# Nikhil-AI-Labs/image-super-resolution-2

Measured on AMD Instinct MI355X. Metric: output MPix/s at x4 SR (256->1024), higher is better.
Workload: dtype bf16 (bf16 MFMA operands, fp32 accumulate, fp32 activations in HBM); 1 GPU; FreqFusion x4 full 3-expert forward (HAT-L + DAT + NAFNet-SR + fusion stack), one 256x256 LR tile -> 1024x1024 per step per GPU (BASELINE configs[1]); seeded synthetic weights (172.3 M params), 1/f-noise tiles; tile=256, parallelism=tile-sharded x1, weights RCCL-broadcast once (0.0 ms), no per-tile collectives, launch=hipGraph replay, tiles_in_flight=2

## Files before the change

### image-super-resolution-2_amd/build.py

```python
from __future__ import annotations

import os
import subprocess
import sys
from concurrent.futures import ThreadPoolExecutor

HERE = os.path.dirname(os.path.abspath(__file__))
CSRC = os.path.join(HERE, "csrc")
LIB = os.path.join(HERE, "libff_hip.so")
SOURCES = ["ff_runtime.hip", "conv_gemm.hip", "conv_gemm_bf16.hip", "conv3x3_halo.hip", "sgfn_tail.hip", "ocab_attn.hip", "conv3x3_small.hip", "attention.hip", "attention_bf16.hip", "win_attn_fused.hip", "chan_qkv.hip", "token_mlp.hip", "token_linear.hip", "naf_fused.hip", "naf_tail.hip", "norm_pool.hip", "dwconv.hip", "elementwise.hip",
           "resample.hip", "freq.hip", "fusion_ops.hip", "metrics.hip", "train_ops.hip", "sr_losses.hip", "augment.hip", "ff_executor.hip"]
HIPCC = os.environ.get("HIPCC", "/opt/rocm/bin/hipcc")
FLAGS = ["--offload-arch=gfx950", "-O3", "-fPIC", "-std=c++17", "-Wall", "-Wno-unused-function", "-I" + os.path.join(HERE, "build")]


def _stale() -> bool:
    if not os.path.exists(LIB):
        return True
    t = os.path.getmtime(LIB)
    deps = [os.path.join(CSRC, f) for f in os.listdir(CSRC)] + [os.path.join(HERE, "..", "include", "ff_kernels.h")]
    return any(os.path.getmtime(d) > t for d in deps)


def gen_dispatch(path: str) -> None:
    from .lib import parse_header
    protos = {n: p for n, p in parse_header().items() if p[1] and p[1][-1] == "void*" and p[0] == "int"
              and n not in ("ff_forward", "ff_create", "ff_upload")}
    names = sorted(protos)
    out = ["// generated by build.py from include/ff_kernels.h -- do not edit", f"#define FF_DISPATCH_COUNT {len(names)}",
           "static const char* const FF_DISPATCH_NAMES[FF_DISPATCH_COUNT] = {" + ", ".join(f'"{n}"' for n in names) + "};"]
    def kinds(n):
        ks = []
        for i, ty in enumerate(protos[n][1]):
            if i == len(protos[n][1]) - 1:
                ks.append("S")
            elif ty.endswith("*"):
                ks.append("P")
            elif ty in ("float", "double"):
                ks.append("F")
            else:
                ks.append("I")
        return "".join(ks)
    out.append("static const char* const FF_DISPATCH_KINDS[FF_DISPATCH_COUNT] = {" + ", ".join(f'"{kinds(n)}"' for n in names) + "};")
# ... 47 lines not shown
```

### image-super-resolution-2_amd/csrc/norm_pool.hip

```cpp
#include "ff_common.h"

template <int NV>
__global__ __launch_bounds__(256) void layernorm_kernel(const float* __restrict__ in, int ldi, float* __restrict__ out,
                                                        int ldo, int rows, int C, const float* __restrict__ g,
                                                        const float* __restrict__ bta, float eps) {
  const int lane = threadIdx.x & 63;
  const int row = blockIdx.x * 4 + (threadIdx.x >> 6);
  if (row >= rows) return;
  const float* x = in + (long long)row * ldi;
  float v[NV];
  float s = 0.f;
#pragma unroll
  for (int i = 0; i < NV; ++i) {
    const int c = lane + 64 * i;
    v[i] = c < C ? x[c] : 0.f;
    s += v[i];
  }
  const float mean = ff_wave_sum(s) / (float)C;
  float q = 0.f;
#pragma unroll
  for (int i = 0; i < NV; ++i) {
    const int c = lane + 64 * i;
    const float d = c < C ? v[i] - mean : 0.f;
    q += d * d;
  }
  const float rstd = 1.0f / sqrtf(ff_wave_sum(q) / (float)C + eps);
  float* y = out + (long long)row * ldo;
#pragma unroll
  for (int i = 0; i < NV; ++i) {
    const int c = lane + 64 * i;
    if (c < C) y[c] = (v[i] - mean) * rstd * g[c] + bta[c];
  }
}

extern "C" int ff_layernorm(const float* in, int ldi, float* out, int ldo, long long rows, int C, const float* gamma,
                            const float* beta, float eps, void* stream) {
  FF_CHECK_ARG(in && out && gamma && beta, "ff_layernorm: null pointer");
  FF_CHECK_ARG(C > 0 && C <= 1024 && ldi >= C && ldo >= C && rows > 0, "ff_layernorm: bad dims C=%d", C);
  FF_CHECK_ARG(rows < (1LL << 31), "ff_layernorm: too many rows");
  hipStream_t st = (hipStream_t)stream;
  dim3 grid((unsigned)((rows + 3) / 4)), block(256);
  const int nv = (C + 63) / 64;
#define LN_CASE(N) hipLaunchKernelGGL(layernorm_kernel<N>, grid, block, 0, st, in, ldi, out, ldo, (int)rows, C, gamma, beta, eps)
  if (nv <= 1) LN_CASE(1);
  else if (nv <= 2) LN_CASE(2);
  else if (nv <= 3) LN_CASE(3);
  else if (nv <= 4) LN_CASE(4);
  else if (nv <= 6) LN_CASE(6);
  else if (nv <= 8) LN_CASE(8);
  else LN_CASE(16);
#undef LN_CASE
  FF_LAUNCH_CHECK("ff_layernorm");
  return FF_OK;
}

__global__ __launch_bounds__(256) void pool_partial_v4_kernel(const float* __restrict__ in, int ld, long long P, int C,
                                                              int pix_per_chunk, float* __restrict__ part) {
  extern __shared__ float4 red4[];
  const int cv = C >> 2, rpi = 256 / cv;
  const int col = threadIdx.x % cv, row = threadIdx.x / cv;
  const int chunk = blockIdx.x, b = blockIdx.y, nch = gridDim.x;
  const long long p0 = (long long)chunk * pix_per_chunk;
  long long p1 = p0 + pix_per_chunk;
  if (p1 > P) p1 = P;
  const float* base = in + (long long)b * P * ld + 4 * col;
  float4 a0 = {0.f, 0.f, 0.f, 0.f}, a1 = a0, a2 = a0, a3 = a0;
  if (row < rpi) {
    long long pp = p0 + row;
    for (; pp + 3LL * rpi < p1; pp += 4LL * rpi) {
      const float4 v0 = *reinterpret_cast<const float4*>(base + pp * ld);
      const float4 v1 = *reinterpret_cast<const float4*>(base + (pp + rpi) * ld);
      const float4 v2 = *reinterpret_cast<const float4*>(base + (pp + 2LL * rpi) * ld);
      const float4 v3 = *reinterpret_cast<const float4*>(base + (pp + 3LL * rpi) * ld);
      a0.x += v0.x; a0.y += v0.y; a0.z += v0.z; a0.w += v0.w;
      a1.x += v1.x; a1.y += v1.y; a1.z += v1.z; a1.w += v1.w;
      a2.x += v2.x; a2.y += v2.y; a2.z += v2.z; a2.w += v2.w;
      a3.x += v3.x; a3.y += v3.y; a3.z += v3.z; a3.w += v3.w;
    }
    for (; pp < p1; pp += rpi) {
      const float4 v0 = *reinterpret_cast<const float4*>(base + pp * ld);
      a0.x += v0.x; a0.y += v0.y; a0.z += v0.z; a0.w += v0.w;
    }
    a0.x += a1.x + a2.x + a3.x; a0.y += a1.y + a2.y + a3.y; a0.z += a1.z + a2.z + a3.z; a0.w += a1.w + a2.w + a3.w;
    red4[row * cv + col] = a0;
  }
  __syncthreads();
// ... 332 lines not shown
```

### image-super-resolution-2_amd/experts.py

```python
from __future__ import annotations

from typing import Dict, List, Optional

import torch

from . import ops
from .prep import (pack_conv, pack_dw, bn_scale_shift, fold_bn_after_conv, pack_token_linear, pack_naf_ffn, pack_naf_tail,
                   pack_win_attn, pack_win_rel, pack_token_projmlp, pack_chan_qkv, pack_token_linear_gated, pack_rel_overlap)

T = torch.Tensor
SD = Dict[str, T]
RGB_MEAN = (0.4488, 0.4371, 0.4040)


def _ceil_to(n: int, m: int) -> int:
    return (n + m - 1) // m * m


class _Weights:

    def __init__(self, sd: SD, dev, prefix: str):
        self.sd, self.dev, self.p = sd, dev, prefix

    def __call__(self, name: str) -> T:
# ... 368 lines not shown
                 dec=(2, 2, 2, 2)):
        w = _Weights(sd, dev, prefix)
        self.dev, self.enc_n, self.mid_n, self.dec_n = dev, enc, mid, dec

        def blk(q):
            def c1(n):
                wt = w(q + n + ".weight")
                return wt.reshape(wt.shape[0], wt.shape[1]).contiguous(), w(q + n + ".bias")
            return dict(n1=(w(q + "norm1.weight"), w(q + "norm1.bias")), n2=(w(q + "norm2.weight"), w(q + "norm2.bias")),
                        c1=c1("conv1"), c2=(pack_dw(w(q + "conv2.weight")), w(q + "conv2.bias")), c3=c1("conv3"),
                        sca=c1("sca.1"), c4=c1("conv4"), c5=c1("conv5"),
                        beta=w(q + "beta").reshape(-1).contiguous(), gamma=w(q + "gamma").reshape(-1).contiguous())

        self.intro = (w.conv("intro"), w("intro.bias"))
        self.ending = (w.conv("ending"), w("ending.bias"))
        self.encs = [[blk(f"encoders.{l}.{b}.") for b in range(n)] for l, n in enumerate(enc)]
        self.mids = [blk(f"middle_blks.{b}.") for b in range(mid)]
        self.decs = [[blk(f"decoders.{l}.{b}.") for b in range(n)] for l, n in enumerate(dec)]
        self.downs = [(w.conv(f"downs.{l}"), w(f"downs.{l}.bias")) for l in range(len(enc))]
        self.ups = [w(f"ups.{l}.0.weight").reshape(w(f"ups.{l}.0.weight").shape[0], -1).contiguous() for l in range(len(dec))]

    def _padded_input(self, B: int, Hp: int, Wp: int, dev) -> T:
        return ops.persistent_zeros(id(self), "naf_in", (B, Hp, Wp, 3), dev)

    def __del__(self):
        try:
            ops.drop_persistent(owner=id(self))
        except Exception:
            pass

    def block(self, x: T, k: dict) -> T:
        c = x.shape[-1]
        flash = ops.fused_modes() and c in (64, 128)
        if flash and c == 64:
            g, pooled = ops.naf_front(x, _tl(k, "c1"), k["n1"][0], k["n1"][1], *k["c2"])
        else:
            if flash:
                t = ops.token_linear(x, _tl(k, "c1"), gamma=k["n1"][0], beta=k["n1"][1], eps=1e-6)
            else:
                t = ops.linear(ops.layernorm(x, *k["n1"], eps=1e-6), *k["c1"])
            g, pooled = ops.dwconv3_gate_pool(t, *k["c2"])
        sca = ops.vec_mlp(pooled, *k["sca"], None)
        if flash and ops.gemm_mode() == "bf16":
            if "tail_pk" not in k:
                k["tail_pk"] = pack_naf_tail(*k["c3"], *k["c4"], *k["c5"])
            return ops.naf_tail(g, x, k["tail_pk"], sca.reshape(-1), k["beta"], k["n2"][0], k["n2"][1], k["gamma"])
        nf = ops.gemm_mode() != "f32"
        if nf:
            y = ops.linear(g, *k["c3"], res=x, mul=k["beta"], kmul=sca.reshape(-1))
        else:
            w3 = ops.mix2(k["c3"][0], ca=sca.reshape(-1))
            y = ops.linear(g, w3, k["c3"][1], res=x, mul=k["beta"], dynamic_w=True)
        if flash:
            if "ffn_pk" not in k:
                k["ffn_pk"] = pack_naf_ffn(k["c4"][0], k["c4"][1], k["c5"][0], k["c5"][1])
            return ops.naf_ffn(y, k["ffn_pk"], k["n2"][0], k["n2"][1], k["gamma"])
        if nf:
            if "c4i" not in k:
                w4, b4 = k["c4"]
                k["c4i"] = (torch.stack((w4[:c], w4[c:]), dim=1).reshape(2 * c, -1).contiguous(),
                            torch.stack((b4[:c], b4[c:]), dim=1).reshape(-1).contiguous())
            g = ops.linear(ops.layernorm(y, *k["n2"], eps=1e-6), *k["c4i"], gate_pairs=True)
        else:
            t = ops.linear(ops.layernorm(y, *k["n2"], eps=1e-6), *k["c4"])
            g = ops.fma3(None, t[..., :c], t[..., c:])
        return ops.linear(g, *k["c5"], res=y, mul=k["gamma"])

    def forward(self, lr: T, taps: Optional[dict] = None, feats: Optional[dict] = None) -> T:
        _, _, h, w = lr.shape
        H, W = 4 * h, 4 * w
        m = 2 ** len(self.enc_n)
        Hp, Wp = _ceil_to(H, m), _ceil_to(W, m)
        inp = self._padded_input(1, Hp, Wp, lr.device)
        ops.resize(lr, (H, W), mode="bicubic", scale_factor=4.0, layout="nchw", out=inp)
        x = ops.conv2d(inp, *self.intro, ksize=(3, 3), pad=(1, 1))
        skips = []
        for lvl, blks in enumerate(self.encs):
            for b, k in enumerate(blks):
                x = self.block(x, k)
                if taps is not None and lvl == 0:
                    taps[f"naf.enc0.b{b}"] = x
            skips.append(x)
            x = ops.conv2d(x, *self.downs[lvl], ksize=(2, 2), stride=(2, 2), pad=(0, 0))
        for k in self.mids:
            x = self.block(x, k)
        if taps is not None:
            taps["naf.mid"] = x
        for lvl, blks in enumerate(self.decs):
            x = ops.conv2d(x, self.ups[lvl], None, shuffle=2, res=skips[-1 - lvl])
            for k in blks:
                x = self.block(x, k)
        if feats is not None:
            feats["nafnet"] = x
        x = ops.conv2d(x, *self.ending, ksize=(3, 3), pad=(1, 1), res=inp)
        return ops.nhwc_to_nchw(x, H, W, clamp01=True)
# ... 1 lines not shown
```

### image-super-resolution-2_amd/ops.py

```python
from __future__ import annotations

from typing import Dict, Optional, Tuple

import torch

from . import lib as _lib

ACT = {None: 0, "none": 0, "gelu": 1, "relu": 2, "lrelu": 3, "sigmoid": 4}
T = torch.Tensor

_PROF = None
_META = [0.0, 0.0]


def _note(flops: float = 0.0, nbytes: float = 0.0):
    _META[0] += flops
    _META[1] += nbytes


def _numel(*ts) -> float:
    return float(sum(t.numel() * (t.element_size() / 4.0) for t in ts if t is not None))


def _instrument(fn):
# ... 37 lines not shown
import os as _os

GEMM_MODES = {"f32": 0, "bf16": 1, "bf16x2": 2, "bf16x3": 3}
_GEMM_MODE = _os.environ.get("FF_GEMM", "bf16x3")


def set_gemm_mode(mode: str):
    global _GEMM_MODE
    if mode not in GEMM_MODES:
        raise _lib.FFError(f"unknown GEMM mode {mode!r}; expected one of {sorted(GEMM_MODES)}")
    _GEMM_MODE = mode


def _nterms() -> int:
    if _GEMM_MODE not in ("bf16x3", "bf16"):
        raise _lib.FFError(f"the fused bf16 kernels exist for the 'bf16x3' and 'bf16' contraction modes, not {_GEMM_MODE!r}")
    return 3 if _GEMM_MODE == "bf16x3" else 1


def fused_modes() -> bool:
    return _GEMM_MODE in ("bf16x3", "bf16")


def gemm_mode() -> str:
    return _GEMM_MODE


_HALO = True


def set_halo(on: bool) -> None:
    global _HALO
    _HALO = bool(on)


def empty_rows_bf16(shape, device) -> T:
    C = int(shape[-1])
    return torch.empty(tuple(shape[:-1]) + ((C + 63) // 64 * 64,), device=device, dtype=torch.bfloat16)[..., :C]


def empty_rows(shape, device) -> T:
    C = int(shape[-1])
    if C >= 48 and C % 32 != 0:
        return torch.empty(tuple(shape[:-1]) + ((C + 31) // 32 * 32,), device=device, dtype=torch.float32)[..., :C]
    return torch.empty(tuple(shape), device=device, dtype=torch.float32)


def empty_like_rows(x: T) -> T:
    return empty_rows(tuple(x.shape), x.device)


_LANE = 0


def lane() -> int:
    return _LANE


def set_lane(k: int) -> None:
    global _LANE
    _LANE = int(k)


_CAPTURE_KEY = None
_PERSIST_GRAPH: Dict[tuple, Dict[tuple, T]] = {}
_PERSIST_EAGER: Dict[tuple, T] = {}
# ... 210 lines not shown

        nt_ = _nterms()

        def _mk_halo():
            bn = _prep.halo_bn(Cout)
            return (_prep.pack_conv3x3_halo(w, Cin, bn, nt_), bn)
        img = PREPARED.get(w, "halo" if nt_ == 3 else "halo1", _mk_halo)
        part = None
        if want_pool and B == 1 and shuffle == 0 and Cout <= img[1]:
            prow = int(_L().ff_conv3x3_halo_pool_rows(B, H, W, Cout, img[1], nt_))
            part = torch.empty((prow, img[1]), device=x.device, dtype=torch.float32)
        _lib.check(_L().ff_conv3x3_halo(xp, ldi, img[0].data_ptr(), img[1], _ptr(bias), _ptr(mul), rp, ldr, op, ldo, B, H, W,
                                        Cin, Cout, ACT[act], float(alpha), shuffle, _ptr(part), _nterms(),
                                        (1 if in_bf16 else 0) | (2 if out_bf16 else 0), _stream()))
        if part is not None:
            pp = PoolPartials(part, Cout, 1.0 / float(H * W))
            _note(2.0 * B * Ho * Wo * Cout * KH * KW * Cin, 4.0 * (_numel(x, w, out, res)))
            return out, (pp if want_pool == "partials" else pp.mean())
    else:
        aligned = (ldi % 4 == 0) and (xp % 16 == 0)
        hi, lo, Kp, Cp, _ = _split_weight(w, dynamic_w, Cin if aligned else 0)
        _lib.check(_L().ff_conv2d_bf16s(xp, hi.data_ptr(), lo.data_ptr() if lo is not None else None, Kp, Cp, _ptr(bias), _ptr(mul),
                                        rp, op, B, H, W, Cin, ldi, Ho, Wo, Cout, ldo, ldr, KH, KW, stride[0], stride[1],
                                        pad[0], pad[1], ACT[act], float(alpha), shuffle, GEMM_MODES[_GEMM_MODE], tile_hint,
                                        None, _stream()))
    _note(2.0 * B * Ho * Wo * Cout * KH * KW * Cin, 4.0 * (_numel(x, w, out, res)))
    if want_pool:
        return out, pool_mean(out)
    return out


def linear(x: T, w: T, bias: Optional[T] = None, *, act=None, res: Optional[T] = None, mul: Optional[T] = None,
           alpha: float = 1.0, out: Optional[T] = None, dynamic_w: bool = False, kmul: Optional[T] = None,
           gate_pairs: bool = False) -> T:
    xp, ldi, rows, K = rows_view(x, "linear.x")
    N = w.shape[0]
    if w.dim() != 2 or w.shape[1] != K or not w.is_contiguous():
        raise _lib.FFError(f"linear: weight must be [N, {K}], got {tuple(w.shape)}")
    if (kmul is not None or gate_pairs) and _GEMM_MODE == "f32":
        raise _lib.FFError("linear: kmul / gate_pairs exist in the split-bf16 kernels only")
    No = N // 2 if gate_pairs else N
    oshape = tuple(x.shape[:-1]) + (No,)
    if out is None:
        out = empty_rows(oshape, x.device)
    op, ldo, orows, oc = rows_view(out, "linear.out")
    if orows != rows or oc != No:
        raise _lib.FFError("linear: out shape mismatch")
    rp, ldr = None, 0
    if res is not None:
        rp, ldr, rrows, rc = rows_view(res, "linear.res")
        if rrows != rows or rc != N:
            raise _lib.FFError("linear: res shape mismatch")
    if _GEMM_MODE == "f32":
        _lib.check(_L().ff_conv2d(xp, w.data_ptr(), _ptr(bias), _ptr(mul), rp, op, 1, 1, rows, K, ldi, 1, rows, N, ldo, ldr,
                                  1, 1, 1, 1, 0, 0, ACT[act], float(alpha), 0, 0, _stream()))
    else:
        aligned = (ldi % 4 == 0) and (xp % 16 == 0)
        hi, lo, Kp, Cp, _ = _split_weight(w, dynamic_w, K if aligned else 0)
        if kmul is not None and (kmul.numel() != K or not kmul.is_contiguous()):
            raise _lib.FFError(f"linear: kmul must be a contiguous [{K}] vector")
        _lib.check(_L().ff_conv2d_bf16s(xp, hi.data_ptr(), lo.data_ptr() if lo is not None else None, Kp, Cp, _ptr(bias), _ptr(mul),
                                        rp, op, 1, 1, rows, K, ldi, 1, rows, N, ldo, ldr, 1, 1, 1, 1, 0, 0, ACT[act],
                                        float(alpha), 1 if gate_pairs else 0, GEMM_MODES[_GEMM_MODE], 0, _ptr(kmul), _stream()))
    _note(2.0 * rows * N * K, 4.0 * (rows * K + N * K + rows * No * (2 if res is not None else 1)))
    return out


def window_attn(qkv: T, out: T, biasT: T, *, q_off: int, k_off: int, v_off: int, o_off: int, H: int, W: int, Hp: int,
                Wp: int, win: Tuple[int, int], kwin: Tuple[int, int], shift: Tuple[int, int], use_mask: bool, heads: int,
                d: int, scale: float, rel_table: Optional[T] = None) -> T:
    qp, ldq, B, h_, w_, _ = _nhwc(qkv, "window_attn.qkv")
    op, ldo, *_ = _nhwc(out, "window_attn.out")
    if (h_, w_) != (H, W) or tuple(out.shape[:3]) != (B, H, W):
        raise _lib.FFError("window_attn: qkv/out spatial dims mismatch")
    nk = kwin[0] * kwin[1]
    if tuple(biasT.shape) != (heads, nk, 256) or not biasT.is_contiguous():
        raise _lib.FFError(f"window_attn: biasT must be [{heads},{nk},256]")
    if q_off + heads * d > qkv.shape[-1] or k_off + heads * d > qkv.shape[-1] or v_off + heads * d > qkv.shape[-1] \
            or o_off + heads * d > out.shape[-1]:
        raise _lib.FFError("window_attn: channel offsets out of range")
    if _GEMM_MODE == "f32":
        _lib.check(_L().ff_window_attn(qp, ldq, q_off, k_off, v_off, op, ldo, o_off, biasT.data_ptr(), B, H, W, Hp, Wp, win[0],
                                       win[1], kwin[0], kwin[1], shift[0], shift[1], int(use_mask), heads, d, float(scale),
                                       _stream()))
    else:
        relp = None
        if rel_table is not None and tuple(kwin) != tuple(win):
            n = (win[0] + kwin[0] - 1) * (win[1] + kwin[1] - 1)
            if tuple(rel_table.shape) != (heads, n) or not rel_table.is_contiguous() or kwin[1] % 8 or tuple(shift) != (0, 0):
                raise _lib.FFError(f"window_attn: overlapping-window rel_table must be [heads, {n}] (prep.pack_rel_overlap), kw % 8 == 0, no shift")
            relp = rel_table.data_ptr()
        elif rel_table is not None and tuple(kwin) == tuple(win) and win[1] & (win[1] - 1) == 0 and win[1] >= 8:
            if tuple(rel_table.shape) != (heads, (2 * win[0] - 1) * (2 * win[1] - 1)) or not rel_table.is_contiguous():
                raise _lib.FFError("window_attn: rel_table must be [heads, (2wh-1)*(2ww-1)]")
            relp = rel_table.data_ptr()
        from . import prep as _prep
        bq = PREPARED.get(biasT, "quad", lambda: _prep.quad_bias(biasT))
# ... 163 lines not shown
    return out, pooled


def naf_ffn(y: T, pk: dict, ln_g: T, ln_b: T, out_scale: T, eps: float = 1e-6) -> T:
    yp, ldy, rows, C = rows_view(y, "naf_ffn.y")
    if C != pk["C"]:
        raise _lib.FFError("naf_ffn: channel mismatch")
    out = torch.empty(tuple(y.shape), device=y.device, dtype=torch.float32)
    _lib.check(_L().ff_naf_ffn(yp, ldy, out.data_ptr(), C, rows, C, ln_g.data_ptr(), ln_b.data_ptr(), float(eps), pk["w"].data_ptr(),
                               pk["b4"].data_ptr(), pk["b5"].data_ptr(), out_scale.data_ptr(), _nterms(), _stream()))
    _note(2.0 * rows * C * 3 * C, 8.0 * rows * C)
    return out


def naf_tail(g: T, x: T, pk: dict, sca: T, beta: T, ln_g: T, ln_b: T, gamma: T, eps: float = 1e-6) -> T:
    if _GEMM_MODE != "bf16":
        raise _lib.FFError(f"naf_tail exists for the plain-bf16 contraction mode only, not {_GEMM_MODE!r}")
    gp, ldg, rows, C = rows_view(g, "naf_tail.g")
    xp, ldx, xr, xc = rows_view(x, "naf_tail.x")
    if C != pk["C"] or xr != rows or xc != C or tuple(x.shape) != tuple(g.shape):
        raise _lib.FFError("naf_tail: shape mismatch")
    for t_, n_ in ((sca, "sca"), (beta, "beta"), (ln_g, "ln_g"), (ln_b, "ln_b"), (gamma, "gamma")):
        _chk(t_, "naf_tail." + n_)
        if t_.numel() != C or not t_.is_contiguous():
            raise _lib.FFError(f"naf_tail: {n_} must be a contiguous [{C}] vector")
    out = torch.empty(tuple(x.shape), device=x.device, dtype=torch.float32)
    _lib.check(_L().ff_naf_tail(gp, ldg, xp, ldx, out.data_ptr(), C, rows, C, sca.data_ptr(), pk["b3"].data_ptr(), beta.data_ptr(),
                                ln_g.data_ptr(), ln_b.data_ptr(), float(eps), pk["w"].data_ptr(), pk["b4"].data_ptr(),
                                pk["b5"].data_ptr(), gamma.data_ptr(), _stream()))
    _note(2.0 * rows * C * 4 * C, 12.0 * rows * C)
    return out


def layernorm(x: T, gamma: T, beta: T, eps: float = 1e-5, out: Optional[T] = None) -> T:
    xp, ldi, rows, C = rows_view(x, "layernorm.x")
    if out is None:
        out = empty_like_rows(x)
    op, ldo, orows, oc = rows_view(out, "layernorm.out")
    if orows != rows or oc != C or gamma.numel() != C or beta.numel() != C:
        raise _lib.FFError("layernorm: shape mismatch")
    _lib.check(_L().ff_layernorm(xp, ldi, op, ldo, rows, C, gamma.data_ptr(), beta.data_ptr(), float(eps), _stream()))
    _note(0.0, 8.0 * rows * C)
    return out


def pool_partials(x: T):
    xp, ld, B, H, W, C = _nhwc(x, "pool_partials.x")
    if B != 1:
        return pool_mean(x)
    P = H * W
    rows = int(_L().ff_pool_partial_rows(P))
    part = torch.empty((rows, C), device=x.device, dtype=torch.float32)
    _lib.check(_L().ff_pool_partials(xp, ld, P, C, part.data_ptr(), part.numel(), _stream()))
    return PoolPartials(part, C, 1.0 / float(P))


def pool_mean(x: T) -> T:
    xp, ld, B, H, W, C = _nhwc(x, "pool_mean.x")
    P = H * W
    nwork = int(_L().ff_pool_mean_workspace(B, P, C))
    work = torch.empty(nwork, device=x.device, dtype=torch.float32)
    out = torch.empty((B, C), device=x.device, dtype=torch.float32)
    _lib.check(_L().ff_pool_mean(xp, ld, B, P, C, out.data_ptr(), work.data_ptr(), nwork, _stream()))
    _note(0.0, 4.0 * B * P * C)
    return out


def vec_mlp(v, W1: T, b1: Optional[T], act1, W2: Optional[T] = None, b2: Optional[T] = None, act2=None,
            post: float = 1.0) -> T:
    if isinstance(v, PoolPartials):
        if W2 is not None and W1.shape[0] <= 64 and v.C <= 512:
            if W1.shape[1] != v.C or W2.shape[1] != W1.shape[0]:
                raise _lib.FFError("vec_mlp: weight shape mismatch")
            out = torch.empty((1, W2.shape[0]), device=v.part.device, dtype=torch.float32)
            _lib.check(_L().ff_pool_vec_mlp(v.part.data_ptr(), v.part.shape[0], v.part.shape[1], v.inv_count, v.C, W1.data_ptr(), _ptr(b1),
# ... 556 lines not shown
```

### include/ff_kernels.h

```cpp
#ifndef FF_KERNELS_H
#define FF_KERNELS_H
#ifdef __cplusplus
extern "C" {
#endif

#define FF_ACT_NONE 0
#define FF_ACT_GELU 1
#define FF_ACT_RELU 2
#define FF_ACT_LRELU 3
#define FF_ACT_SIGMOID 4

const char* ff_last_error(void);
int ff_abi_version(void);
int ff_device_cu_count(void);

int ff_conv2d(const float* in, const float* w, const float* bias, const float* mul, const float* res, float* out,
              int B, int H, int W, int Cin, int ldi, int Ho, int Wo, int Cout, int ldo, int ldr, int KH, int KW,
              int sy, int sx, int py, int px, int act, float alpha, int shuffle, int tile_hint, void* stream);

int ff_conv2d_bf16s(const float* in, const void* w_hi, const void* w_lo, int Kp, int Cp, const float* bias, const float* mul,
                    const float* res, float* out, int B, int H, int W, int Cin, int ldi, int Ho, int Wo, int Cout,
                    int ldo, int ldr, int KH, int KW, int sy, int sx, int py, int px, int act, float alpha, int shuffle,
                    int nterms, int tile_hint, const float* kmul, void* stream);
int ff_split_bf16(const float* w, int N, int K, int Kp, int Cin, int Cp, void* hi, void* lo, void* stream);

int ff_conv3x3_small(const float* in, int ldi, const float* w_small, int ct, const float* bias, const float* res, int ldr,
                     float* out, int ldo, int B, int H, int W, int Cin, int Cout, int act, float alpha, void* stream);


int ff_window_attn(const float* qkv, int ldq, int q_off, int k_off, int v_off, float* out, int ldo, int o_off,
                   const float* biasT, int B, int H, int W, int Hp, int Wp, int wh, int ww, int kh, int kw,
                   int shift_h, int shift_w, int use_mask, int heads, int d, float scale, void* stream);

int ff_window_attn_bf16s(const float* qkv, int ldq, int q_off, int k_off, int v_off, float* out, int ldo, int o_off,
                         const float* biasT, int B, int H, int W, int Hp, int Wp, int wh, int ww, int kh, int kw,
                         int shift_h, int shift_w, int use_mask, int heads, int d, float scale, int nterms, const float* rel_table,
                         void* stream);

int ff_token_projmlp(const float* att, int lda, const float* x, int ldx, const float* c2, int ldc, const float* c2_scale,
                     float* out, int ldo, long long M, int K, int hidden_tiles, const void* proj_tiles,
                     const float* proj_bias_padded, const float* gamma, const float* beta, float eps,
                     const void* mlp_tiles, const float* b1_padded, const float* b2, int nterms, int io_bf16, void* stream);

int ff_win_attn_fused(const float* x, int ldx, float* out, int ldo, int o_off, const float* gamma, const float* beta,
                      float eps, const void* w_tiles, const float* bias_padded, const float* rel_padded, int rel_rows,
                      int rel_stride, int B, int H, int W, int Hp, int Wp, int wh, int ww, int shift_h, int shift_w,
                      int use_mask, int head0, int nheads, int d, int K, int zero_pad_tokens, float* xn_out, int ldxn,
                      float* v_out, int ldv, int v_off, int nterms, int out_bf16, int xn_bf16, void* stream);

int ff_token_mlp(const float* x, int ldx, float* out, int ldo, long long M, int K, int hidden_tiles, int N,
                 const float* gamma, const float* beta, float eps, const void* w_tiles, const float* b1_padded,
                 const float* b2, int nterms, void* stream);

long long ff_conv3x3_halo_weight_bytes(int Cout, int Cin, int bn, int nterms);
long long ff_conv3x3_halo_pool_rows(int B, int H, int W, int Cout, int bn, int nterms);
int ff_pool_finish(const float* part, int rows, int ld, int C, float inv_count, float* out, void* stream);
int ff_conv3x3_halo(const float* in, int ldi, const void* w_img, int bn, const float* bias, const float* mul,
                    const float* res, int ldr, float* out, int ldo, int B, int H, int W, int Cin, int Cout,
                    int act, float alpha, int shuffle, float* pool_partials, int nterms, int io_bf16, void* stream);

int ff_token_linear(const float* x, int ldx, float* out, int ldo, long long M, int K, int kpad, int N, int n_tiles,
                    const float* gamma, const float* beta, float eps, const void* w_tiles, const float* bias_padded,
                    int act, const float* res, int ldr, const float* res2, int ldr2, const float* res2_scale,
                    float* xn_out, int ldxn, float* stats_out, int stat_lo,
                    int stat_hi, float stat_eps, int nterms, void* stream);

int ff_token_linear_gated(const float* x, int ldx, const float* x2, int ldx2, const float* cm, const float* gw1t, const float* gb1,
                          const float* gw2, float gb2, float* out, int ldo, long long M, int K, int N, int n_tiles,
                          const void* w_tiles, const float* bias_padded, const float* res, int ldr, int nterms, void* stream);

long long ff_dwconv3_gate_pool_workspace(int C);
int ff_dwconv3_gate_pool(const float* in, int ldi, float* out, int ldo, int H, int W, int C, const float* w_tapmajor,
                         const float* bias, float* pooled, float* work, long long work_floats, void* stream);

long long ff_naf_front_workspace(int H, int W, int C);
int ff_naf_front(const float* x, int ldx, int H, int W, int C, const float* ln_gamma, const float* ln_beta, float eps,
                 const void* w1_tiles, const float* b1, const float* dw_tapmajor, const float* dw_bias, float* out, int ldo,
                 float* pooled, float* work, long long work_floats, int nterms, void* stream);
int ff_naf_ffn(const float* y, int ldy, float* out, int ldo, long long M, int C, const float* gamma_ln, const float* beta_ln,
               float eps, const void* w_tiles, const float* b4, const float* b5, const float* out_scale, int nterms, void* stream);

int ff_naf_tail(const float* g, int ldg, const float* x, int ldx, float* out, int ldo, long long M, int C, const float* sca,
                const float* b3, const float* beta, const float* gamma_ln, const float* beta_ln, float eps, const void* w_frags,
                const float* b4, const float* b5, const float* out_scale, void* stream);

int ff_layernorm(const float* in, int ldi, float* out, int ldo, long long rows, int C, const float* gamma,
                 const float* beta, float eps, void* stream);

int ff_pool_mean(const float* in, int ld, int B, long long P, int C, float* out, float* work, long long work_floats,
                 void* stream);
long long ff_pool_mean_workspace(int B, long long P, int C);

int ff_vec_mlp(const float* in, int B, int Cin, const float* W1, const float* b1, int Ch, int act1, const float* W2,
               const float* b2, int Cout, int act2, float post, float* out, void* stream);

int ff_pool_partial_rows(long long P);
int ff_pool_partials(const float* in, int ld, long long P, int C, float* part, long long part_floats, void* stream);

int ff_pool_vec_mlp(const float* part, int rows, int ld, float inv_count, int Cin, const float* W1, const float* b1, int Ch,
                    int act1, const float* W2, const float* b2, int Cout, int act2, float post, float* out, float* pooled_out,
                    void* stream);

int ff_ocab_attn(const float* qkv, int ldq, int q_off, int k_off, int v_off, float* out, int ldo, int o_off,
                 const float* rel_rotated, int B, int H, int W, int heads, int d, int ws, int ows, float scale, int out_bf16, void* stream);

int ff_sgfn_tail(const float* h, int ldh, int c2, const float* stats, const float* gamma, const float* beta,
                 const float* dw_tapmajor, const float* dw_bias, const void* fc2_tiles, int hidden_tiles, const float* b2,
                 const float* res, int ldr, float* out, int ldo, int B, int H, int W, int N, void* stream);

int ff_dwconv2d(const float* in, int ldi, float* out, int ldo, int B, int H, int W, int C, int Ho, int Wo,
                const float* w_tapmajor, const float* bias, int KH, int KW, int sy, int sx, int py, int px,
                const float* post_scale, const float* post_shift, int act, const float* mul_in, int ldm, void* stream);

int ff_dwconv3x3_ln(const float* in, int ldi, float* out, int ldo, int B, int H, int W, int C, const float* w_tapmajor,
                    const float* bias, const float* stats, const float* gamma, const float* beta, const float* mul_in, int ldm,
                    void* stream);

int ff_mix2(float* out, int ldo, const float* a, int lda, const float* b, int ldb, long long rows, int C, float ka,
            float kb, const float* ca, const float* cb, const float* pa, int ldpa, const float* pb, int ldpb,
            int clamp01, void* stream);
// ... 147 lines not shown
```

Measured before the change: 24.72 output MPix/s.

## Add bf16-row GEMM path for NAFNet non-flash blocks with bf16 LayerNorm outputs

Result: faster. 25.91 output MPix/s (median of 6 runs) (+4.8%).

```diff
diff --git a/image-super-resolution-2_amd/build.py b/image-super-resolution-2_amd/build.py
--- a/image-super-resolution-2_amd/build.py
+++ b/image-super-resolution-2_amd/build.py
@@ -8,7 +8,7 @@
 HERE = os.path.dirname(os.path.abspath(__file__))
 CSRC = os.path.join(HERE, "csrc")
 LIB = os.path.join(HERE, "libff_hip.so")
-SOURCES = ["ff_runtime.hip", "conv_gemm.hip", "conv_gemm_bf16.hip", "conv3x3_halo.hip", "sgfn_tail.hip", "ocab_attn.hip", "conv3x3_small.hip", "attention.hip", "attention_bf16.hip", "win_attn_fused.hip", "chan_qkv.hip", "token_mlp.hip", "token_linear.hip", "naf_fused.hip", "naf_tail.hip", "norm_pool.hip", "dwconv.hip", "elementwise.hip",
+SOURCES = ["ff_runtime.hip", "conv_gemm.hip", "conv_gemm_bf16.hip", "gemm_rows_bf16.hip", "conv3x3_halo.hip", "sgfn_tail.hip", "ocab_attn.hip", "conv3x3_small.hip", "attention.hip", "attention_bf16.hip", "win_attn_fused.hip", "chan_qkv.hip", "token_mlp.hip", "token_linear.hip", "naf_fused.hip", "naf_tail.hip", "norm_pool.hip", "dwconv.hip", "elementwise.hip",
            "resample.hip", "freq.hip", "fusion_ops.hip", "metrics.hip", "train_ops.hip", "sr_losses.hip", "augment.hip", "ff_executor.hip"]
 HIPCC = os.environ.get("HIPCC", "/opt/rocm/bin/hipcc")
 FLAGS = ["--offload-arch=gfx950", "-O3", "-fPIC", "-std=c++17", "-Wall", "-Wno-unused-function", "-I" + os.path.join(HERE, "build")]
diff --git a/image-super-resolution-2_amd/csrc/gemm_rows_bf16.hip b/image-super-resolution-2_amd/csrc/gemm_rows_bf16.hip
--- /dev/null
+++ b/image-super-resolution-2_amd/csrc/gemm_rows_bf16.hip
@@ -0,0 +1,245 @@
+#include "ff_common.h"
+
+struct RowsGemmParams {
+  const void* a;
+  const float* kmul;
+  const __bf16* w;
+  const float* bias;
+  const float* mul;
+  const float* res;
+  void* out;
+  int M, N, K;
+  int lda, ldo, ldr;
+};
+
+template <int BM, int BN, int WM, int WN, bool GATE, bool A32>
+__global__ __launch_bounds__(WM * WN * 64) void gemm_rows_bf16_kernel(RowsGemmParams p) {
+  constexpr int NW = WM * WN;
+  constexpr int TM = BM / WM, TN = BN / WN;
+  constexpr int MI = TM / 32, NI = TN / 32;
+  constexpr int AI = A32 ? 0 : BM / 8 / NW, BI = BN / 8 / NW;
+  constexpr int AS = A32 ? BM / (8 * NW) : 0;
+  constexpr int ABYTES = BM * 128, BUFB = (BM + BN) * 128;
+  static_assert(BM % (8 * NW) == 0 && BN % (8 * NW) == 0, "DMA pieces must tile the waves");
+  extern __shared__ __attribute__((aligned(16))) unsigned char smem[];
+
+  const int tid = threadIdx.x;
+  const int lane = tid & 63, wid = tid >> 6;
+  const int l31 = lane & 31, hh = lane >> 5;
+  const int wr = wid / WN, wc = wid % WN;
+
+  const int mtiles = (p.M + BM - 1) / BM, ntiles = (p.N + BN - 1) / BN;
+  const int L = ff_xcd_remap(blockIdx.x, mtiles * ntiles);
+  const int m0 = (L / ntiles) * BM, n0 = (L % ntiles) * BN;
+
+  const __bf16* asrc[AI + 1];
+  const __bf16* bsrc[BI];
+#pragma unroll
+  for (int i = 0; i < AI; ++i) {
+    const int row = 8 * (wid + NW * i) + (lane >> 3);
+    const int q = (lane & 7) ^ ((row >> 1) & 7);
+    const int m = m0 + row < p.M ? m0 + row : p.M - 1;
+    asrc[i] = reinterpret_cast<const __bf16*>(p.a) + (long long)m * p.lda + 8 * q;
+  }
+  const float* fsrc[AS + 1];
+  int fdst[AS + 1];
+  f32x4 ra[AS + 1][2], km[2];
+#pragma unroll
+  for (int i = 0; i < AS; ++i) {
+    const int row = (tid >> 3) + 8 * NW * i, q = tid & 7;
+    const int m = m0 + row < p.M ? m0 + row : p.M - 1;
+    fsrc[i] = reinterpret_cast<const float*>(p.a) + (long long)m * p.lda + 8 * q;
+    fdst[i] = row * 128 + (q ^ ((row >> 1) & 7)) * 16;
+  }
+  auto load_a = [&](int c) {
+#pragma unroll
+    for (int i = 0; i < AS; ++i) {
+      ra[i][0] = *reinterpret_cast<const f32x4*>(fsrc[i] + 64 * c);
+      ra[i][1] = *reinterpret_cast<const f32x4*>(fsrc[i] + 64 * c + 4);
+    }
+    if (p.kmul) {
+      km[0] = *reinterpret_cast<const f32x4*>(p.kmul + 64 * c + 8 * (tid & 7));
+      km[1] = *reinterpret_cast<const f32x4*>(p.kmul + 64 * c + 8 * (tid & 7) + 4);
+    }
+  };
+  auto store_a = [&](int buf) {
+#pragma unroll
+    for (int i = 0; i < AS; ++i) {
+      f32x4 u = ra[i][0], v = ra[i][1];
+      if (p.kmul) { u *= km[0]; v *= km[1]; }
+      const bf16x8 h = {(__bf16)u[0], (__bf16)u[1], (__bf16)u[2], (__bf16)u[3], (__bf16)v[0], (__bf16)v[1], (__bf16)v[2], (__bf16)v[3]};
+      *reinterpret_cast<bf16x8*>(smem + buf * BUFB + fdst[i]) = h;
+    }
+  };
+#pragma unroll
+  for (int i = 0; i < BI; ++i) {
+    const int row = 8 * (wid + NW * i) + (lane >> 3);
+    const int q = (lane & 7) ^ ((row >> 1) & 7);
+    const int n = n0 + row < p.N ? n0 + row : p.N - 1;
+    bsrc[i] = p.w + (long long)n * p.K + 8 * q;
+  }
+  auto dma = [&](int c, int buf) {
+    unsigned char* dst = smem + buf * BUFB;
+#pragma unroll
+    for (int i = 0; i < AI; ++i)
+      __builtin_amdgcn_global_load_lds((const __attribute__((address_space(1))) void*)(asrc[i] + 64 * c),
+                                       (__attribute__((address_space(3))) void*)(dst + (wid + NW * i) * 1024), 16, 0, 0);
+#pragma unroll
+    for (int i = 0; i < BI; ++i)
+      __builtin_amdgcn_global_load_lds((const __attribute__((address_space(1))) void*)(bsrc[i] + 64 * c),
+                                       (__attribute__((address_space(3))) void*)(dst + ABYTES + (wid + NW * i) * 1024), 16, 0, 0);
+  };
+
+  f32x16 acc[MI][NI];
+#pragma unroll
+  for (int i = 0; i < MI; ++i)
+#pragma unroll
+    for (int j = 0; j < NI; ++j)
+#pragma unroll
+      for (int r = 0; r < 16; ++r) acc[i][j][r] = 0.f;
+
+  const int sw = (l31 >> 1) & 7;
+  const int arow = (wr * TM + l31) * 128, brow = ABYTES + (wc * TN + l31) * 128;
+  const int nchunks = p.K / 64;
+  if (A32) load_a(0);
+  dma(0, 0);
+  for (int c = 0; c < nchunks; ++c) {
+    const int buf = c & 1;
+    if (A32) store_a(buf);
+    asm volatile("s_waitcnt vmcnt(0)" ::: "memory");
+    __syncthreads();
+    if (c + 1 < nchunks) {
+      if (A32) load_a(c + 1);
+      dma(c + 1, buf ^ 1);
+    }
+    const unsigned char* base = smem + buf * BUFB;
+#pragma unroll
+    for (int s = 0; s < 4; ++s) {
+      const int slot = ((2 * s + hh) ^ sw) * 16;
+      bf16x8 a[MI], b[NI];
+#pragma unroll
+      for (int i = 0; i < MI; ++i) a[i] = *reinterpret_cast<const bf16x8*>(base + arow + i * 32 * 128 + slot);
+#pragma unroll
+      for (int j = 0; j < NI; ++j) b[j] = *reinterpret_cast<const bf16x8*>(base + brow + j * 32 * 128 + slot);
+#pragma unroll
+      for (int i = 0; i < MI; ++i)
+#pragma unroll
+        for (int j = 0; j < NI; ++j) acc[i][j] = __builtin_amdgcn_mfma_f32_32x32x16_bf16(a[i], b[j], acc[i][j], 0, 0, 0);
+    }
+  }
+  __syncthreads();
+
+  float* tr = reinterpret_cast<float*>(smem) + wid * (32 * 36);
+  if (GATE) {
+    __bf16* out = reinterpret_cast<__bf16*>(p.out);
+    const int grow = lane >> 2, seg = lane & 3;
+#pragma unroll
+    for (int j = 0; j < NI; ++j) {
+      const int n = n0 + wc * TN + j * 32 + l31;
+      const float bv = (p.bias && n < p.N) ? p.bias[n] : 0.f;
+      const int nq = (n0 + wc * TN + j * 32) / 2 + 4 * seg;
+      const bool nqok = nq < p.N / 2;
+#pragma unroll
+      for (int i = 0; i < MI; ++i) {
+        const int mb = m0 + wr * TM + i * 32;
+#pragma unroll
+        for (int r = 0; r < 16; ++r) tr[((r & 3) + 8 * (r >> 2) + 4 * hh) * 36 + l31] = acc[i][j][r] + bv;
+#pragma unroll
+        for (int pass = 0; pass < 2; ++pass) {
+          const int row = grow + 16 * pass;
+          const f32x4 a = *reinterpret_cast<const f32x4*>(tr + row * 36 + 8 * seg);
+          const f32x4 b2 = *reinterpret_cast<const f32x4*>(tr + row * 36 + 8 * seg + 4);
+          const f32x4 o = {a[0] * a[1], a[2] * a[3], b2[0] * b2[1], b2[2] * b2[3]};
+          const bf16x4 ob = {(__bf16)o[0], (__bf16)o[1], (__bf16)o[2], (__bf16)o[3]};
+          const int m = mb + row;
+          if (nqok && m < p.M) *reinterpret_cast<bf16x4*>(out + (long long)m * p.ldo + nq) = ob;
+        }
+      }
+    }
+  } else {
+    float* out = reinterpret_cast<float*>(p.out);
+    const bool has_res = p.res != nullptr;
+    const int tq = lane >> 3, q4 = 4 * (lane & 7);
+#pragma unroll
+    for (int j = 0; j < NI; ++j) {
+      const int n = n0 + wc * TN + j * 32 + l31;
+      const int nc = n < p.N ? n : 0;
+      const float bv = p.bias ? p.bias[nc] : 0.f;
+      const float mv = p.mul ? p.mul[nc] : 1.f;
+      const int nq = n0 + wc * TN + j * 32 + q4;
+      const bool nqok = nq < p.N;
+#pragma unroll
+      for (int i = 0; i < MI; ++i) {
+        const int mb = m0 + wr * TM + i * 32;
+        f32x4 rq[4];
+        long long oo[4];
+        bool ok[4];
+#pragma unroll
+        for (int k = 0; k < 4; ++k) {
+          const int m = mb + tq + 8 * k;
+          ok[k] = nqok && m < p.M;
+          oo[k] = ok[k] ? (long long)m * p.ldo + nq : 0;
+          f32x4 r0 = {0.f, 0.f, 0.f, 0.f};
+          if (has_res) { const f32x4 u = *reinterpret_cast<const f32x4*>(p.res + (ok[k] ? (long long)m * p.ldr + nq : 0)); r0 = ok[k] ? u : r0; }
+          rq[k] = r0;
+        }
+#pragma unroll
+        for (int r = 0; r < 16; ++r) tr[((r & 3) + 8 * (r >> 2) + 4 * hh) * 36 + l31] = (acc[i][j][r] + bv) * mv;
+        f32x4 ov[4];
+#pragma unroll
+        for (int k = 0; k < 4; ++k) ov[k] = *reinterpret_cast<const f32x4*>(tr + (tq + 8 * k) * 36 + q4) + rq[k];
+#pragma unroll
+        for (int k = 0; k < 4; ++k)
+          if (ok[k]) *reinterpret_cast<f32x4*>(out + oo[k]) = ov[k];
+      }
+    }
+  }
+}
+
+template <int BM, int BN, int WM, int WN>
+static int launch_rows(const RowsGemmParams& p, bool gate, bool a32, hipStream_t st) {
+  constexpr size_t lds = (size_t)2 * (BM + BN) * 128;
+  static_assert(lds <= 64 * 1024 && lds >= (size_t)WM * WN * 32 * 36 * 4, "LDS budget (two staging buffers; the epilogue patches reuse them)");
+  dim3 grid((unsigned)(ff_cdiv(p.M, BM) * ff_cdiv(p.N, BN))), block(WM * WN * 64);
+  if (a32)
+    hipLaunchKernelGGL((gemm_rows_bf16_kernel<BM, BN, WM, WN, false, true>), grid, block, lds, st, p);
+  else if (gate)
+    hipLaunchKernelGGL((gemm_rows_bf16_kernel<BM, BN, WM, WN, true, false>), grid, block, lds, st, p);
+  else
+    hipLaunchKernelGGL((gemm_rows_bf16_kernel<BM, BN, WM, WN, false, false>), grid, block, lds, st, p);
+  FF_LAUNCH_CHECK("ff_gemm_rows_bf16");
+  return FF_OK;
+}
+
+extern "C" int ff_gemm_rows_bf16(const void* a, int a_fp32, int lda, const void* w_hi, int Kp, const float* kmul, const float* bias,
+                                 const float* mul, const float* res, int ldr, void* out, int ldo, long long M, int N, int K, int gate,
+                                 int tile_hint, void* stream) {
+  FF_CHECK_ARG(a && w_hi && out, "ff_gemm_rows_bf16: null pointer");
+  FF_CHECK_ARG(M > 0 && M < (1LL << 31) && N > 0 && K > 0, "ff_gemm_rows_bf16: bad dims");
+  FF_CHECK_ARG(K % 64 == 0 && Kp == K, "ff_gemm_rows_bf16: needs K %% 64 == 0 and an unpadded weight plane (Kp == K), got K=%d Kp=%d", K, Kp);
+  FF_CHECK_ARG(a_fp32 == 0 || a_fp32 == 1, "ff_gemm_rows_bf16: a_fp32 must be 0 or 1");
+  FF_CHECK_ARG(lda >= K && lda % (a_fp32 ? 4 : 8) == 0 && (((uintptr_t)a) & 15) == 0 && (((uintptr_t)w_hi) & 15) == 0,
+               "ff_gemm_rows_bf16: A rows and the weight plane must be 16-byte aligned (lda %% 8 == 0, fp32 rows lda %% 4 == 0; lda >= K)");
+  FF_CHECK_ARG(gate == 0 || gate == 1, "ff_gemm_rows_bf16: gate must be 0 or 1");
+  FF_CHECK_ARG(!a_fp32 || !gate, "ff_gemm_rows_bf16: fp32 A rows come with the fp32-rows epilogue only");
+  FF_CHECK_ARG(!kmul || (a_fp32 && (((uintptr_t)kmul) & 15) == 0), "ff_gemm_rows_bf16: kmul scales fp32 A rows only and must be 16-byte aligned");
+  if (gate) {
+    FF_CHECK_ARG(N % 8 == 0 && !res && !mul && ldo >= N / 2 && ldo % 4 == 0 && (((uintptr_t)out) & 7) == 0,
+                 "ff_gemm_rows_bf16: the pair-product epilogue needs N %% 8 == 0, no residual / scale and 8-byte aligned bf16 output rows");
+  } else {
+    FF_CHECK_ARG(N % 4 == 0 && ldo >= N && ldo % 4 == 0 && (((uintptr_t)out) & 15) == 0,
+                 "ff_gemm_rows_bf16: needs N %% 4 == 0 and 16-byte aligned output rows");
+    FF_CHECK_ARG(!res || (ldr >= N && ldr % 4 == 0 && (((uintptr_t)res) & 15) == 0), "ff_gemm_rows_bf16: residual rows must be 16-byte aligned");
+  }
+  RowsGemmParams p;
+  p.a = a; p.kmul = kmul; p.w = (const __bf16*)w_hi; p.bias = bias; p.mul = mul; p.res = res; p.out = out;
+  p.M = (int)M; p.N = N; p.K = K; p.lda = lda; p.ldo = ldo; p.ldr = ldr;
+  hipStream_t st = (hipStream_t)stream;
+  int cfg = tile_hint;
+  if (cfg <= 0) cfg = ff_cdiv(M, 128) * ff_cdiv(N, 128) <= 256 ? 2 : 1;
+  switch (cfg) {
+    case 1: return launch_rows<128, 128, 2, 4>(p, gate != 0, a_fp32 != 0, st);
+    case 2: return launch_rows<128, 64, 4, 2>(p, gate != 0, a_fp32 != 0, st);
+    default: ff_set_error("ff_gemm_rows_bf16: bad tile_hint %d", cfg); return FF_ERR_ARG;
+  }
+}
diff --git a/image-super-resolution-2_amd/csrc/norm_pool.hip b/image-super-resolution-2_amd/csrc/norm_pool.hip
--- a/image-super-resolution-2_amd/csrc/norm_pool.hip
+++ b/image-super-resolution-2_amd/csrc/norm_pool.hip
@@ -1,7 +1,7 @@
 #include "ff_common.h"
 
-template <int NV>
-__global__ __launch_bounds__(256) void layernorm_kernel(const float* __restrict__ in, int ldi, float* __restrict__ out,
+template <int NV, bool BF16OUT>
+__global__ __launch_bounds__(256) void layernorm_kernel(const float* __restrict__ in, int ldi, void* __restrict__ out,
                                                         int ldo, int rows, int C, const float* __restrict__ g,
                                                         const float* __restrict__ bta, float eps) {
   const int lane = threadIdx.x & 63;
@@ -25,23 +25,27 @@
     q += d * d;
   }
   const float rstd = 1.0f / sqrtf(ff_wave_sum(q) / (float)C + eps);
-  float* y = out + (long long)row * ldo;
 #pragma unroll
   for (int i = 0; i < NV; ++i) {
     const int c = lane + 64 * i;
-    if (c < C) y[c] = (v[i] - mean) * rstd * g[c] + bta[c];
-  }
-}
-
-extern "C" int ff_layernorm(const float* in, int ldi, float* out, int ldo, long long rows, int C, const float* gamma,
+    if (c < C) {
+      const float yv = (v[i] - mean) * rstd * g[c] + bta[c];
+      if (BF16OUT) reinterpret_cast<__bf16*>(out)[(long long)row * ldo + c] = (__bf16)yv;
+      else reinterpret_cast<float*>(out)[(long long)row * ldo + c] = yv;
+    }
+  }
+}
+
+template <bool BF16OUT>
+static int layernorm_launch(const char* name, const float* in, int ldi, void* out, int ldo, long long rows, int C, const float* gamma,
                             const float* beta, float eps, void* stream) {
-  FF_CHECK_ARG(in && out && gamma && beta, "ff_layernorm: null pointer");
-  FF_CHECK_ARG(C > 0 && C <= 1024 && ldi >= C && ldo >= C && rows > 0, "ff_layernorm: bad dims C=%d", C);
-  FF_CHECK_ARG(rows < (1LL << 31), "ff_layernorm: too many rows");
+  FF_CHECK_ARG(in && out && gamma && beta, "%s: null pointer", name);
+  FF_CHECK_ARG(C > 0 && C <= 1024 && ldi >= C && ldo >= C && rows > 0, "%s: bad dims C=%d", name, C);
+  FF_CHECK_ARG(rows < (1LL << 31), "%s: too many rows", name);
   hipStream_t st = (hipStream_t)stream;
   dim3 grid((unsigned)((rows + 3) / 4)), block(256);
   const int nv = (C + 63) / 64;
-#define LN_CASE(N) hipLaunchKernelGGL(layernorm_kernel<N>, grid, block, 0, st, in, ldi, out, ldo, (int)rows, C, gamma, beta, eps)
+#define LN_CASE(N) hipLaunchKernelGGL((layernorm_kernel<N, BF16OUT>), grid, block, 0, st, in, ldi, out, ldo, (int)rows, C, gamma, beta, eps)
   if (nv <= 1) LN_CASE(1);
   else if (nv <= 2) LN_CASE(2);
   else if (nv <= 3) LN_CASE(3);
@@ -50,8 +54,18 @@
   else if (nv <= 8) LN_CASE(8);
   else LN_CASE(16);
 #undef LN_CASE
-  FF_LAUNCH_CHECK("ff_layernorm");
-  return FF_OK;
+  FF_LAUNCH_CHECK(name);
+  return FF_OK;
+}
+
+extern "C" int ff_layernorm(const float* in, int ldi, float* out, int ldo, long long rows, int C, const float* gamma,
+                            const float* beta, float eps, void* stream) {
+  return layernorm_launch<false>("ff_layernorm", in, ldi, out, ldo, rows, C, gamma, beta, eps, stream);
+}
+
+extern "C" int ff_layernorm_bf16out(const float* in, int ldi, void* out, int ldo, long long rows, int C, const float* gamma,
+                                    const float* beta, float eps, void* stream) {
+  return layernorm_launch<true>("ff_layernorm_bf16out", in, ldi, out, ldo, rows, C, gamma, beta, eps, stream);
 }
 
 __global__ __launch_bounds__(256) void pool_partial_v4_kernel(const float* __restrict__ in, int ld, long long P, int C,
diff --git a/image-super-resolution-2_amd/experts.py b/image-super-resolution-2_amd/experts.py
--- a/image-super-resolution-2_amd/experts.py
+++ b/image-super-resolution-2_amd/experts.py
@@ -424,13 +424,14 @@
     def block(self, x: T, k: dict) -> T:
         c = x.shape[-1]
         flash = ops.fused_modes() and c in (64, 128)
+        rows = not flash and ops.gemm_mode() == "bf16" and ops.rows_gemm() and ops.rows_gemm_ok(c)
         if flash and c == 64:
             g, pooled = ops.naf_front(x, _tl(k, "c1"), k["n1"][0], k["n1"][1], *k["c2"])
         else:
             if flash:
                 t = ops.token_linear(x, _tl(k, "c1"), gamma=k["n1"][0], beta=k["n1"][1], eps=1e-6)
             else:
-                t = ops.linear(ops.layernorm(x, *k["n1"], eps=1e-6), *k["c1"])
+                t = ops.linear(ops.layernorm(x, *k["n1"], eps=1e-6, out_bf16=rows), *k["c1"])
             g, pooled = ops.dwconv3_gate_pool(t, *k["c2"])
         sca = ops.vec_mlp(pooled, *k["sca"], None)
         if flash and ops.gemm_mode() == "bf16":
@@ -439,7 +440,7 @@
             return ops.naf_tail(g, x, k["tail_pk"], sca.reshape(-1), k["beta"], k["n2"][0], k["n2"][1], k["gamma"])
         nf = ops.gemm_mode() != "f32"
         if nf:
-            y = ops.linear(g, *k["c3"], res=x, mul=k["beta"], kmul=sca.reshape(-1))
+            y = ops.linear(g, *k["c3"], res=x, mul=k["beta"], kmul=sca.reshape(-1), rows_gemm=rows)
         else:
             w3 = ops.mix2(k["c3"][0], ca=sca.reshape(-1))
             y = ops.linear(g, w3, k["c3"][1], res=x, mul=k["beta"], dynamic_w=True)
@@ -452,7 +453,7 @@
                 w4, b4 = k["c4"]
                 k["c4i"] = (torch.stack((w4[:c], w4[c:]), dim=1).reshape(2 * c, -1).contiguous(),
                             torch.stack((b4[:c], b4[c:]), dim=1).reshape(-1).contiguous())
-            g = ops.linear(ops.layernorm(y, *k["n2"], eps=1e-6), *k["c4i"], gate_pairs=True)
+            g = ops.linear(ops.layernorm(y, *k["n2"], eps=1e-6, out_bf16=rows), *k["c4i"], gate_pairs=True, out_bf16=rows)
         else:
             t = ops.linear(ops.layernorm(y, *k["n2"], eps=1e-6), *k["c4"])
             g = ops.fma3(None, t[..., :c], t[..., c:])
diff --git a/image-super-resolution-2_amd/ops.py b/image-super-resolution-2_amd/ops.py
--- a/image-super-resolution-2_amd/ops.py
+++ b/image-super-resolution-2_amd/ops.py
@@ -93,6 +93,18 @@
 def set_halo(on: bool) -> None:
     global _HALO
     _HALO = bool(on)
+
+
+_ROWS_GEMM = True
+
+
+def set_rows_gemm(on: bool) -> None:
+    global _ROWS_GEMM
+    _ROWS_GEMM = bool(on)
+
+
+def rows_gemm() -> bool:
+    return _ROWS_GEMM
 
 
 def empty_rows_bf16(shape, device) -> T:
@@ -369,7 +381,12 @@
 
 def linear(x: T, w: T, bias: Optional[T] = None, *, act=None, res: Optional[T] = None, mul: Optional[T] = None,
            alpha: float = 1.0, out: Optional[T] = None, dynamic_w: bool = False, kmul: Optional[T] = None,
-           gate_pairs: bool = False) -> T:
+           gate_pairs: bool = False, out_bf16: bool = False, tile_hint: int = 0, rows_gemm: bool = False) -> T:
+    if x.dtype == torch.bfloat16 or rows_gemm:
+        return _linear_rows_bf16(x, w, bias, act=act, res=res, mul=mul, alpha=alpha, out=out, dynamic_w=dynamic_w, kmul=kmul,
+                                 gate_pairs=gate_pairs, out_bf16=out_bf16, tile_hint=tile_hint)
+    if out_bf16 or tile_hint:
+        raise _lib.FFError("linear: out_bf16 / tile_hint belong to the bf16-rows route (bf16 x, or rows_gemm)")
     xp, ldi, rows, K = rows_view(x, "linear.x")
     N = w.shape[0]
     if w.dim() != 2 or w.shape[1] != K or not w.is_contiguous():
@@ -400,6 +417,44 @@
                                         rp, op, 1, 1, rows, K, ldi, 1, rows, N, ldo, ldr, 1, 1, 1, 1, 0, 0, ACT[act],
                                         float(alpha), 1 if gate_pairs else 0, GEMM_MODES[_GEMM_MODE], 0, _ptr(kmul), _stream()))
     _note(2.0 * rows * N * K, 4.0 * (rows * K + N * K + rows * No * (2 if res is not None else 1)))
+    return out
+
+
+def rows_gemm_ok(K: int) -> bool:
+    return K % 64 == 0
+
+
+def _linear_rows_bf16(x: T, w: T, bias, *, act, res, mul, alpha, out, dynamic_w, kmul, gate_pairs, out_bf16, tile_hint) -> T:
+    xp, lda, rows, K = rows_view(x, "linear.x|bf16ok")
+    a32 = x.dtype == torch.float32
+    N = w.shape[0]
+    if w.dim() != 2 or w.shape[1] != K or not w.is_contiguous():
+        raise _lib.FFError(f"linear: weight must be [N, {K}], got {tuple(w.shape)}")
+    if _GEMM_MODE != "bf16" or not rows_gemm_ok(K):
+        raise _lib.FFError("linear: the bf16-rows GEMM exists in plain-bf16 mode for K % 64 == 0 only")
+    if kmul is not None and (not a32 or kmul.numel() != K or not kmul.is_contiguous()):
+        raise _lib.FFError(f"linear: kmul scales fp32 input rows only and must be a contiguous [{K}] vector")
+    if act is not None or alpha != 1.0 or (a32 and gate_pairs) or (gate_pairs and (res is not None or mul is not None)) or out_bf16 != gate_pairs:
+        raise _lib.FFError("linear: the bf16-rows GEMM has three epilogues: bias (* mul + res) -> fp32 rows, or the SimpleGate pair "
+                           "product -> bf16 rows")
+    No = N // 2 if gate_pairs else N
+    oshape = tuple(x.shape[:-1]) + (No,)
+    if out is None:
+        out = empty_rows_bf16(oshape, x.device) if out_bf16 else empty_rows(oshape, x.device)
+    elif (out.dtype == torch.bfloat16) != out_bf16:
+        raise _lib.FFError("linear: out dtype does not match out_bf16")
+    op, ldo, orows, oc = rows_view(out, "linear.out|bf16ok" if out_bf16 else "linear.out")
+    if orows != rows or oc != No:
+        raise _lib.FFError("linear: out shape mismatch")
+    rp, ldr = None, 0
+    if res is not None:
+        rp, ldr, rrows, rc = rows_view(res, "linear.res")
+        if rrows != rows or rc != N:
+            raise _lib.FFError("linear: res shape mismatch")
+    hi, _, Kp, _, _ = _split_weight(w, dynamic_w, K)
+    _lib.check(_L().ff_gemm_rows_bf16(xp, 1 if a32 else 0, lda, hi.data_ptr(), Kp, _ptr(kmul), _ptr(bias), _ptr(mul), rp, ldr, op, ldo, rows,
+                                      N, K, 1 if gate_pairs else 0, int(tile_hint), _stream()))
+    _note(2.0 * rows * N * K, (4.0 if a32 else 2.0) * rows * K + 2.0 * N * K + (2.0 if out_bf16 else 4.0) * rows * No + (4.0 * rows * No if res is not None else 0.0))
     return out
 
 
@@ -629,15 +684,18 @@
     return out
 
 
-def layernorm(x: T, gamma: T, beta: T, eps: float = 1e-5, out: Optional[T] = None) -> T:
+def layernorm(x: T, gamma: T, beta: T, eps: float = 1e-5, out: Optional[T] = None, out_bf16: bool = False) -> T:
     xp, ldi, rows, C = rows_view(x, "layernorm.x")
     if out is None:
-        out = empty_like_rows(x)
-    op, ldo, orows, oc = rows_view(out, "layernorm.out")
+        out = empty_rows_bf16(tuple(x.shape), x.device) if out_bf16 else empty_like_rows(x)
+    elif (out.dtype == torch.bfloat16) != out_bf16:
+        raise _lib.FFError("layernorm: out dtype does not match out_bf16")
+    op, ldo, orows, oc = rows_view(out, "layernorm.out|bf16ok" if out_bf16 else "layernorm.out")
     if orows != rows or oc != C or gamma.numel() != C or beta.numel() != C:
         raise _lib.FFError("layernorm: shape mismatch")
-    _lib.check(_L().ff_layernorm(xp, ldi, op, ldo, rows, C, gamma.data_ptr(), beta.data_ptr(), float(eps), _stream()))
-    _note(0.0, 8.0 * rows * C)
+    fn = _L().ff_layernorm_bf16out if out_bf16 else _L().ff_layernorm
+    _lib.check(fn(xp, ldi, op, ldo, rows, C, gamma.data_ptr(), beta.data_ptr(), float(eps), _stream()))
+    _note(0.0, (6.0 if out_bf16 else 8.0) * rows * C)
     return out
 
 
diff --git a/include/ff_kernels.h b/include/ff_kernels.h
--- a/include/ff_kernels.h
+++ b/include/ff_kernels.h
@@ -23,6 +23,10 @@
                     int ldo, int ldr, int KH, int KW, int sy, int sx, int py, int px, int act, float alpha, int shuffle,
                     int nterms, int tile_hint, const float* kmul, void* stream);
 int ff_split_bf16(const float* w, int N, int K, int Kp, int Cin, int Cp, void* hi, void* lo, void* stream);
+
+int ff_gemm_rows_bf16(const void* a, int a_fp32, int lda, const void* w_hi, int Kp, const float* kmul, const float* bias,
+                      const float* mul, const float* res, int ldr, void* out, int ldo, long long M, int N, int K, int gate,
+                      int tile_hint, void* stream);
 
 int ff_conv3x3_small(const float* in, int ldi, const float* w_small, int ct, const float* bias, const float* res, int ldr,
                      float* out, int ldo, int B, int H, int W, int Cin, int Cout, int act, float alpha, void* stream);
@@ -86,6 +90,8 @@
 
 int ff_layernorm(const float* in, int ldi, float* out, int ldo, long long rows, int C, const float* gamma,
                  const float* beta, float eps, void* stream);
+int ff_layernorm_bf16out(const float* in, int ldi, void* out, int ldo, long long rows, int C, const float* gamma,
+                         const float* beta, float eps, void* stream);
 
 int ff_pool_mean(const float* in, int ld, int B, long long P, int C, float* out, float* work, long long work_floats,
                  void* stream);
```
